# CIAM-Group/ComputerVision_Codes

Hardware: AMD Instinct MI355X
Metric: frames/sec spatial-extract + per-video TCN latency, Cholec80, 1/2/4/8 GPU (higher is better)
Workload: dtype bf16

## Files before the change

### computervision_codes_amd/csrc/bottleneck_fused.hip

```cpp
#include "mt4_common.h"

typedef __bf16 bf16x8_t __attribute__((ext_vector_type(8)));

namespace {

constexpr int TH = 8, TW = 14, NHALO = 160, NPX = 128;
constexpr int ROW_B = 128;
constexpr int XS_BYTES = NHALO * ROW_B;
constexpr int T2_BYTES = NPX * ROW_B;
constexpr int T1_BYTES = XS_BYTES + 2 * ROW_B;
constexpr int YS_BYTES = NPX * 256;

struct BneckK {
    const char* x;
    char* y;
    const char *w1, *w2, *w3, *wds;
    const float *b1, *b2, *b3, *bds;
    int B, H, W, tiles_h, tiles_w;
    int nt;
    char* y2;
    const char* wn;
    const float* bn;
    int H2, W2;
};

__device__ __forceinline__ f32x4 bias4(const float* b, int n) {
    const float4 t = *(const float4*)(b + n);
    return (f32x4){t.x, t.y, t.z, t.w};
}

__device__ __forceinline__ uint2 relu_pack4(f32x4 v) {
    uint2 o = make_uint2(pack_bf16x2(v[0], v[1]), pack_bf16x2(v[2], v[3]));
    asm("v_pk_max_i16 %0, %0, 0" : "+v"(o.x));
    asm("v_pk_max_i16 %0, %0, 0" : "+v"(o.y));
    return o;
}

__device__ __forceinline__ f32x4 mfma_bf16(uint4 wfrag, uint4 xfrag, f32x4 acc) {
    return __builtin_amdgcn_mfma_f32_16x16x32_bf16(__builtin_bit_cast(bf16x8_t, wfrag), __builtin_bit_cast(bf16x8_t, xfrag), acc, 0, 0, 0);
}

template <int CIN, bool DS, bool NEXT = false>
__global__ __launch_bounds__(256, 2) void bottleneck64_fused_kernel(const BneckK a) {
    static_assert(!NEXT || !DS, "the following conv rides behind an identity block");
    constexpr int KC = CIN / 64;
    constexpr int NXS = KC > 1 ? 2 : 1;
    static_assert(DS ? CIN == 64 : CIN == 256, "layer1.0 (64 channels in, downsample branch) or layer1.1+ (256 in, identity)");
    extern __shared__ __attribute__((aligned(16))) char smem[];
    char* const xs = smem;
    char* const t2 = smem + NXS * XS_BYTES;
    char* const t1 = t2 + T2_BYTES;
    char* const ys = DS ? t1 : xs;

    const int tid = threadIdx.x;
    const int lane = tid & 63, wave = tid >> 6;
    const int r16 = lane & 15, q = lane >> 4;

    int bid = blockIdx.x;
    {
        const int nb = gridDim.x;
        const int q8 = nb >> 3, r8 = nb & 7;
        const int xcd = bid & 7, local = bid >> 3;
        bid = (xcd < r8 ? xcd * (q8 + 1) : r8 * (q8 + 1) + (xcd - r8) * q8) + local;
    }
    const int tpi = a.tiles_h * a.tiles_w;
    const int img = bid / tpi;
    const int trem = bid - img * tpi;
    const int th = trem / a.tiles_w;
    const int h0 = th * TH, w0 = (trem - th * a.tiles_w) * TW;
    const char* const ximg = a.x + (long long)img * a.H * a.W * (CIN * 2);
    char* const yimg = NEXT ? a.y + (long long)img * a.H2 * a.W2 * 512 : a.y + (long long)img * a.H * a.W * 512;

    const int ld_row = tid >> 3, ld_chunk = tid & 7;
    int xoff[5];
#pragma unroll
    for (int i = 0; i < 5; ++i) {
        const int hp = ld_row + 32 * i;
        const int h = h0 - 1 + (hp >> 4), w = w0 - 1 + (hp & 15);
        xoff[i] = ((unsigned)h < (unsigned)a.H && (unsigned)w < (unsigned)a.W) ? (h * a.W + w) * (CIN * 2) + ld_chunk * 16 : -1;
    }
    auto load_chunk = [&](int kc, uint4 (&stg)[5]) {
#pragma unroll
        for (int i = 0; i < 5; ++i) {
            stg[i] = make_uint4(0, 0, 0, 0);
            if (xoff[i] >= 0) stg[i] = *(const uint4*)(ximg + xoff[i] + kc * 128);
        }
    };
    auto store_chunk = [&](int buf, const uint4 (&stg)[5]) {
#pragma unroll
        for (int i = 0; i < 5; ++i) {
            const int hp = ld_row + 32 * i;
            *(uint4*)(xs + buf * XS_BYTES + hp * ROW_B + ((ld_chunk ^ (hp & 7)) << 4)) = stg[i];
        }
    };
    uint4 stg0[5], stg1[5];
    load_chunk(0, stg0);
    if constexpr (KC > 1) load_chunk(1, stg1);

    const int ch1 = wave * 16;
    uint4 wf1[KC * 2];
    {
        const char* wr = a.w1 + (wave * (KC * 2) * 64 + lane) * 16;
#pragma unroll
        for (int s = 0; s < KC * 2; ++s) wf1[s] = *(const uint4*)(wr + s * 1024);
    }
    f32x4 acc1[10];
    {
        const f32x4 b4 = bias4(a.b1, ch1 + q * 4);
#pragma unroll
        for (int i = 0; i < 10; ++i) acc1[i] = b4;
    }
    const int sw0 = (q ^ (r16 & 7)) << 4, sw1 = ((4 + q) ^ (r16 & 7)) << 4;
    uint2 res[DS ? 1 : 4][DS ? 1 : 8];
    const int res_off = (r16 + 1) * ROW_B + (((2 * wave + (q >> 1)) ^ ((r16 + 1) & 7)) << 4) + (q & 1) * 8;
#pragma unroll
    for (int kc = 0; kc < KC; ++kc) {
        if (kc & 1) store_chunk(1, stg1); else store_chunk(0, stg0);
        if (kc + 2 < KC) { if (kc & 1) load_chunk(kc + 2, stg1); else load_chunk(kc + 2, stg0); }
        __syncthreads();
        const char* sb = xs + (kc & 1) * XS_BYTES + r16 * ROW_B;
        uint4 fx[2][10];
#pragma unroll
        for (int kk = 0; kk < 2; ++kk)
#pragma unroll
            for (int i = 0; i < 10; ++i) fx[kk][i] = *(const uint4*)(sb + i * 16 * ROW_B + (kk ? sw1 : sw0));
        if constexpr (!DS) {
#pragma unroll
            for (int j = 0; j < 8; ++j) res[kc][j] = *(const uint2*)(xs + (kc & 1) * XS_BYTES + (j + 1) * (16 * ROW_B) + res_off);
        }
        asm volatile("" ::: "memory");
#pragma unroll
        for (int kk = 0; kk < 2; ++kk)
#pragma unroll
            for (int i = 0; i < 10; ++i) acc1[i] = mfma_bf16(wf1[kc * 2 + kk], fx[kk][i], acc1[i]);
    }
    uint4 wf2[18];
    {
        const char* wr = a.w2 + (wave * 18 * 64 + lane) * 16;
#pragma unroll
        for (int s = 0; s < 18; ++s) wf2[s] = *(const uint4*)(wr + s * 1024);
    }
    const int cb1 = (ch1 + q * 4) * 2;
    {
        const int wr_off = r16 * ROW_B + (((cb1 >> 4) ^ (r16 & 7)) << 4) + (cb1 & 8);
        const int w = w0 - 1 + r16;
#pragma unroll
        for (int i = 0; i < 10; ++i) {
            const int h = h0 - 1 + i;
            const bool in = (unsigned)h < (unsigned)a.H && (unsigned)w < (unsigned)a.W;
            uint2 o = make_uint2(0, 0);
            if (in) o = relu_pack4(acc1[i]);
            *(uint2*)(t1 + i * (16 * ROW_B) + wr_off) = o;
        }
    }
    __syncthreads();

    f32x4 acc2[8];
    {
        const f32x4 b4 = bias4(a.b2, ch1 + q * 4);
#pragma unroll
        for (int j = 0; j < 8; ++j) acc2[j] = b4;
    }
    int toff[3][2];
#pragma unroll
    for (int kw = 0; kw < 3; ++kw)
#pragma unroll
        for (int kk = 0; kk < 2; ++kk) toff[kw][kk] = (r16 + kw) * ROW_B + (((kk * 4 + q) ^ ((r16 + kw) & 7)) << 4);
#pragma unroll
    for (int hr = 0; hr < 10; ++hr) {
        uint4 fr[3][2];
#pragma unroll
        for (int kw = 0; kw < 3; ++kw)
#pragma unroll
            for (int kk = 0; kk < 2; ++kk) fr[kw][kk] = *(const uint4*)(t1 + hr * (16 * ROW_B) + toff[kw][kk]);
        asm volatile("" ::: "memory");
#pragma unroll
        for (int kh = 0; kh < 3; ++kh) {
            const int ty = hr - kh;
            if (ty >= 0 && ty < 8) {
#pragma unroll
                for (int kw = 0; kw < 3; ++kw)
#pragma unroll
                    for (int kk = 0; kk < 2; ++kk) acc2[ty] = mfma_bf16(wf2[(kh * 3 + kw) * 2 + kk], fr[kw][kk], acc2[ty]);
            }
        }
    }
    uint4 wf3[4][2];
    uint4 wfd[DS ? 4 : 1][2];
#pragma unroll
    for (int i = 0; i < 4; ++i) {
        const char* wr = a.w3 + ((4 * i + wave) * 2 * 64 + lane) * 16;
        wf3[i][0] = *(const uint4*)wr;
        wf3[i][1] = *(const uint4*)(wr + 1024);
        if constexpr (DS) {
            const char* wd = a.wds + ((4 * i + wave) * 2 * 64 + lane) * 16;
            wfd[i][0] = *(const uint4*)wd;
            wfd[i][1] = *(const uint4*)(wd + 1024);
        }
    }
    {
        const int wr_off = r16 * ROW_B + (((cb1 >> 4) ^ (r16 & 7)) << 4) + (cb1 & 8);
#pragma unroll
        for (int j = 0; j < 8; ++j) {
            const uint2 o = relu_pack4(acc2[j]);
            *(uint2*)(t2 + j * (16 * ROW_B) + wr_off) = o;
        }
    }
    __syncthreads();

    uint4 fx3[8][2];
#pragma unroll
    for (int j = 0; j < 8; ++j) {
        fx3[j][0] = *(const uint4*)(t2 + j * (16 * ROW_B) + r16 * ROW_B + sw0);
        fx3[j][1] = *(const uint4*)(t2 + j * (16 * ROW_B) + r16 * ROW_B + sw1);
    }
    const int st_tx = tid >> 4, st_chunk = tid & 15;
    uint4 wfn[NEXT ? 2 : 1][NEXT ? 8 : 1];
#pragma unroll
    for (int pass = 0; pass < 2; ++pass) {
        char* const ysp = NEXT ? xs + pass * YS_BYTES : ys;
        if (pass && !NEXT) __syncthreads();
#pragma unroll
        for (int ii = 0; ii < 2; ++ii) {
            const int i = pass * 2 + ii;
            const int ct = 4 * i + wave;
            f32x4 acc3[8];
            {
                const f32x4 b4 = bias4(a.b3, ct * 16 + q * 4);
#pragma unroll
                for (int j = 0; j < 8; ++j) acc3[j] = b4;
            }
#pragma unroll
            for (int kk = 0; kk < 2; ++kk)
#pragma unroll
                for (int j = 0; j < 8; ++j) acc3[j] = mfma_bf16(wf3[i][kk], fx3[j][kk], acc3[j]);
            if constexpr (DS) {
                const f32x4 bd4 = bias4(a.bds, ct * 16 + q * 4);
#pragma unroll
                for (int j = 0; j < 8; ++j) {
                    f32x4 accd = bd4;
#pragma unroll
                    for (int kk = 0; kk < 2; ++kk) accd = mfma_bf16(wfd[i][kk], *(const uint4*)(xs + (j + 1) * (16 * ROW_B) + toff[1][kk]), accd);
#pragma unroll
                    for (int e = 0; e < 4; ++e) acc3[j][e] += bf16_to_f32(f32_to_bf16(accd[e]));
                }
            } else {
#pragma unroll
                for (int j = 0; j < 8; ++j) {
                    acc3[j][0] += __uint_as_float(res[i][j].x << 16);
                    acc3[j][1] += __uint_as_float(res[i][j].x & 0xffff0000u);
                    acc3[j][2] += __uint_as_float(res[i][j].y << 16);
                    acc3[j][3] += __uint_as_float(res[i][j].y & 0xffff0000u);
                }
            }
            const int cbyte = ((ct - 8 * pass) * 16 + q * 4) * 2;
            const int wr_off = r16 * 256 + (((cbyte >> 4) ^ r16) << 4) + (cbyte & 8);
#pragma unroll
            for (int j = 0; j < 8; ++j) {
                const uint2 o = relu_pack4(acc3[j]);
                *(uint2*)(ysp + j * (16 * 256) + wr_off) = o;
            }
        }
        if constexpr (NEXT) {
            if (pass == 1) {
#pragma unroll
                for (int c = 0; c < 2; ++c)
#pragma unroll
                    for (int ks = 0; ks < 8; ++ks) wfn[c][ks] = *(const uint4*)(a.wn + (((2 * wave + c) * 8 + ks) * 64 + lane) * 16);
            }
        }
        __syncthreads();
        {
            const int w = w0 + st_tx;
            const int rd_off = st_tx * 256 + ((st_chunk ^ st_tx) << 4);
            if constexpr (NEXT) {
                if (st_tx < TW && w < a.W && !(st_tx & 1)) {
                    const uint4 v0 = *(const uint4*)(ysp + rd_off), v1 = *(const uint4*)(ysp + 2 * (16 * 256) + rd_off);
                    const uint4 v2 = *(const uint4*)(ysp + 4 * (16 * 256) + rd_off), v3 = *(const uint4*)(ysp + 6 * (16 * 256) + rd_off);
                    char* const yp = yimg + (unsigned)(((h0 >> 1) * a.W2 + (w >> 1)) * 512 + pass * 256 + st_chunk * 16);
                    const int rows = a.H - h0;
                    *(uint4*)yp = v0;
                    if (rows > 2) *(uint4*)(yp + a.W2 * 512) = v1;
                    if (rows > 4) *(uint4*)(yp + 2 * a.W2 * 512) = v2;
                    if (rows > 6) *(uint4*)(yp + 3 * a.W2 * 512) = v3;
                }
            } else if (st_tx < TW && w < a.W) {
                uint4 v[8];
#pragma unroll
                for (int ty = 0; ty < 8; ++ty) v[ty] = *(const uint4*)(ysp + ty * (16 * 256) + rd_off);
                asm volatile("" ::: "memory");
#pragma unroll
                for (int ty = 0; ty < 8; ++ty) {
                    if (h0 + ty < a.H) {
                        typedef unsigned u32x4 __attribute__((ext_vector_type(4)));
                        char* yp = yimg + (unsigned)((h0 + ty) * a.W * 512) + (unsigned)(w * 512 + pass * 256 + st_chunk * 16);
                        if (a.nt) __builtin_nontemporal_store((u32x4){v[ty].x, v[ty].y, v[ty].z, v[ty].w}, (u32x4*)yp);
                        else *(uint4*)yp = v[ty];
                    }
                }
            }
        }
    }
    if constexpr (NEXT) {
        f32x4 acc4[2][8];
#pragma unroll
        for (int c = 0; c < 2; ++c) {
            const f32x4 b4 = bias4(a.bn, (2 * wave + c) * 16 + q * 4);
#pragma unroll
            for (int j = 0; j < 8; ++j) acc4[c][j] = b4;
        }
#pragma unroll
        for (int ks = 0; ks < 8; ++ks) {
            uint4 fy[8];
            const char* yb = xs + (ks >> 2) * YS_BYTES + r16 * 256 + ((((ks & 3) * 4 + q) ^ r16) << 4);
#pragma unroll
            for (int j = 0; j < 8; ++j) fy[j] = *(const uint4*)(yb + j * (16 * 256));
            asm volatile("" ::: "memory");
#pragma unroll
            for (int c = 0; c < 2; ++c)
#pragma unroll
                for (int j = 0; j < 8; ++j) acc4[c][j] = mfma_bf16(wfn[c][ks], fy[j], acc4[c][j]);
        }
        __syncthreads();
#pragma unroll
        for (int c = 0; c < 2; ++c) {
            const int cbyte = ((2 * wave + c) * 16 + q * 4) * 2;
            const int wr_off = r16 * 256 + (((cbyte >> 4) ^ r16) << 4) + (cbyte & 8);
#pragma unroll
            for (int j = 0; j < 8; ++j) *(uint2*)(xs + j * (16 * 256) + wr_off) = relu_pack4(acc4[c][j]);
        }
        __syncthreads();
        const int w = w0 + st_tx;
        if (st_tx < TW && w < a.W) {
            const int rd_off = st_tx * 256 + ((st_chunk ^ st_tx) << 4);
            char* const y2img = a.y2 + (long long)img * a.H * a.W * 256;
            uint4 v[8];
#pragma unroll
            for (int ty = 0; ty < 8; ++ty) v[ty] = *(const uint4*)(xs + ty * (16 * 256) + rd_off);
            asm volatile("" ::: "memory");
#pragma unroll
            for (int ty = 0; ty < 8; ++ty) {
                if (h0 + ty < a.H) {
                    typedef unsigned u32x4 __attribute__((ext_vector_type(4)));
                    char* yp = y2img + (unsigned)(((h0 + ty) * a.W + w) * 256 + st_chunk * 16);
                    if (a.nt) __builtin_nontemporal_store((u32x4){v[ty].x, v[ty].y, v[ty].z, v[ty].w}, (u32x4*)yp);
                    else *(uint4*)yp = v[ty];
                }
            }
        }
    }
}

template <int CIN, bool DS, bool NEXT = false>
int launch(const BneckK& a, hipStream_t stream) {
    constexpr int NXS = CIN > 64 ? 2 : 1;
    constexpr int LDS = NXS * XS_BYTES + T2_BYTES + (DS ? YS_BYTES : T1_BYTES);
    static_assert(LDS <= 80 * 1024, "two workgroups per CU");
    static_assert(!NEXT || LDS >= 2 * YS_BYTES, "both output passes stay in LDS");
    auto fn = bottleneck64_fused_kernel<CIN, DS, NEXT>;
    MT4_RAISE_LDS(fn);
    const long long nblk = (long long)a.B * a.tiles_h * a.tiles_w;
    hipLaunchKernelGGL(fn, dim3((unsigned)nblk), dim3(256), LDS, stream, a);
    return mt4_check_launch();
}

}

__global__ void bneck_pack_kernel(const u16* __restrict__ w, uint4* __restrict__ out, int ctiles, int ksteps, int row_elems) {
    const int i = blockIdx.x * blockDim.x + threadIdx.x;
    if (i >= ctiles * ksteps * 64) return;
    const int lane = i & 63, fs = i >> 6;
    const int step = fs % ksteps, tile = fs / ksteps;
    out[i] = *(const uint4*)(w + (long long)(tile * 16 + (lane & 15)) * row_elems + step * 32 + (lane >> 4) * 8);
}

static inline long long bneck_frag_bytes(int Cin, bool ds) { return ((long long)4 * (Cin / 32) + 4 * 18 + 16 * 2 + (ds ? 16 * (Cin / 32) : 0)) * 1024; }

extern "C" int64_t mt4_bottleneck_packed_bytes(int32_t Cin, int32_t has_downsample) {
    if (!((has_downsample && Cin == 64) || (!has_downsample && Cin == 256))) return MT4_EUNSUPPORTED;
    return bneck_frag_bytes(Cin, has_downsample != 0);
}

extern "C" int mt4_bottleneck_pack_bf16(const void* w1, const void* w2, const void* w3, const void* wds, int32_t Cin, void* out, void* stream) {
    mt4_clear_error();
    if (!w1 || !w2 || !w3 || !out) return MT4_EINVAL;
    if (!((wds && Cin == 64) || (!wds && Cin == 256))) return MT4_EUNSUPPORTED;
    if (((uintptr_t)w1 | (uintptr_t)w2 | (uintptr_t)w3 | (uintptr_t)wds | (uintptr_t)out) & 15) return MT4_EALIGN;
    hipStream_t s = (hipStream_t)stream;
    const int k1 = Cin / 32;
    char* o = (char*)out;
    const int r1 = (int)mt4_conv_packed_k(Cin, 1, 1, MT4_BF16), r2 = (int)mt4_conv_packed_k(64, 3, 3, MT4_BF16), r3 = (int)mt4_conv_packed_k(64, 1, 1, MT4_BF16);
    auto go = [&](const void* w, int ctiles, int ksteps, int row_elems) {
        const int n = ctiles * ksteps * 64;
        hipLaunchKernelGGL(bneck_pack_kernel, dim3((n + 255) / 256), dim3(256), 0, s, (const u16*)w, (uint4*)o, ctiles, ksteps, row_elems);
        o += (long long)n * 16;
    };
    go(w1, 4, k1, r1);
    go(w2, 4, 18, r2);
    go(w3, 16, 2, r3);
    if (wds) go(wds, 16, k1, r1);
    return mt4_check_launch();
}

extern "C" int mt4_bottleneck_fused_bf16(const void* x, void* y, const void* w_frag, const float* b1, const float* b2, const float* b3, const float* bds,
                                         int32_t B, int32_t H, int32_t W, int32_t Cin, int32_t mid, void* stream) {
    mt4_clear_error();
    if (!x || !y || !w_frag || !b1 || !b2 || !b3 || B <= 0 || H <= 0 || W <= 0) return MT4_EINVAL;
    const bool ds = bds != nullptr;
    if (mid != 64 || !((ds && Cin == 64) || (!ds && Cin == 256))) return MT4_EUNSUPPORTED;
    if (((uintptr_t)x | (uintptr_t)y | (uintptr_t)w_frag | (uintptr_t)b1 | (uintptr_t)b2 | (uintptr_t)b3 | (uintptr_t)bds) & 15) return MT4_EALIGN;
    if ((long long)H * W * 512 > 0x7fffffffLL) return MT4_EUNSUPPORTED;
    BneckK a;
    a.x = (const char*)x; a.y = (char*)y;
    const int k1 = Cin / 32;
    a.w1 = (const char*)w_frag;
    a.w2 = a.w1 + (long long)4 * k1 * 1024;
    a.w3 = a.w2 + (long long)4 * 18 * 1024;
    a.wds = ds ? a.w3 + (long long)16 * 2 * 1024 : nullptr;
    a.b1 = b1; a.b2 = b2; a.b3 = b3; a.bds = bds;
    a.B = B; a.H = H; a.W = W;
    a.tiles_h = cdiv(H, TH); a.tiles_w = cdiv(W, TW);
    a.nt = 1;
    if ((long long)B * a.tiles_h * a.tiles_w > 0x7fffffffLL) return MT4_EUNSUPPORTED;
    return ds ? launch<64, true>(a, (hipStream_t)stream) : launch<256, false>(a, (hipStream_t)stream);
}

extern "C" int64_t mt4_bottleneck_next_packed_bytes(void) { return (int64_t)8 * 8 * 1024; }

extern "C" int mt4_bottleneck_pack_next_bf16(const void* w1_next, void* out, void* stream) {
    mt4_clear_error();
    if (!w1_next || !out) return MT4_EINVAL;
    if (((uintptr_t)w1_next | (uintptr_t)out) & 15) return MT4_EALIGN;
    const int n = 8 * 8 * 64;
    hipLaunchKernelGGL(bneck_pack_kernel, dim3((n + 255) / 256), dim3(256), 0, (hipStream_t)stream, (const u16*)w1_next, (uint4*)out, 8, 8,
                       (int)mt4_conv_packed_k(256, 1, 1, MT4_BF16));
    return mt4_check_launch();
}

extern "C" int mt4_bottleneck_fused_next_bf16(const void* x, void* y_even, void* t_next, const void* w_frag, const float* b1, const float* b2,
                                              const float* b3, const void* w_next, const float* b_next, int32_t B, int32_t H, int32_t W, void* stream) {
    mt4_clear_error();
    if (!x || !y_even || !t_next || !w_frag || !b1 || !b2 || !b3 || !w_next || !b_next || B <= 0 || H <= 0 || W <= 0) return MT4_EINVAL;
    if (((uintptr_t)x | (uintptr_t)y_even | (uintptr_t)t_next | (uintptr_t)w_frag | (uintptr_t)b1 | (uintptr_t)b2 | (uintptr_t)b3 | (uintptr_t)w_next |
         (uintptr_t)b_next) & 15)
        return MT4_EALIGN;
    if ((long long)H * W * 512 > 0x7fffffffLL) return MT4_EUNSUPPORTED;
    BneckK a{};
    a.x = (const char*)x; a.y = (char*)y_even; a.y2 = (char*)t_next;
    a.w1 = (const char*)w_frag;
    a.w2 = a.w1 + (long long)4 * 8 * 1024;
    a.w3 = a.w2 + (long long)4 * 18 * 1024;
    a.wds = nullptr;
    a.b1 = b1; a.b2 = b2; a.b3 = b3; a.bds = nullptr;
    a.wn = (const char*)w_next; a.bn = b_next;
    a.B = B; a.H = H; a.W = W; a.H2 = (H + 1) / 2; a.W2 = (W + 1) / 2;
    a.tiles_h = cdiv(H, TH); a.tiles_w = cdiv(W, TW);
    a.nt = 1;
    if ((long long)B * a.tiles_h * a.tiles_w > 0x7fffffffLL) return MT4_EUNSUPPORTED;
    return launch<256, false, true>(a, (hipStream_t)stream);
}

extern "C" int mt4_pack_fragments_bf16(const void* w_packed, int32_t rows, int32_t row_elems, void* out, void* stream) {
    mt4_clear_error();
    if (!w_packed || !out || rows <= 0 || row_elems <= 0) return MT4_EINVAL;
    if ((rows % 16) || (row_elems % 32)) return MT4_EUNSUPPORTED;
    if (((uintptr_t)w_packed | (uintptr_t)out) & 15) return MT4_EALIGN;
    const long long n = (long long)(rows / 16) * (row_elems / 32) * 64;
    if (n > 0x7fffffffLL) return MT4_EUNSUPPORTED;
    hipLaunchKernelGGL(bneck_pack_kernel, dim3((unsigned)((n + 255) / 256)), dim3(256), 0, (hipStream_t)stream, (const u16*)w_packed, (uint4*)out, rows / 16,
                       row_elems / 32, row_elems);
    return mt4_check_launch();
}
```

Before: 97370.

## Process vertical strips of tiles per workgroup, carrying conv1 halo rows between bands

Each workgroup now walks a vertical strip of up to several 8x14 tiles instead of one tile. The two halo rows of the 1x1 conv output and the residual row are carried in LDS and registers to the next band, so recomputing the halo conv1 rows and reloading the overlapping input rows is avoided. It reduces the redundant 10-vs-8 row work and the halo reads, at the cost of fewer workgroups (with a floor of 1024 blocks), more serialization per block and extra LDS for the DS variant.

```diff
diff --git a/computervision_codes_amd/csrc/bottleneck_fused.hip b/computervision_codes_amd/csrc/bottleneck_fused.hip
--- a/computervision_codes_amd/csrc/bottleneck_fused.hip
+++ b/computervision_codes_amd/csrc/bottleneck_fused.hip
@@ -17,6 +17,7 @@
     const char *w1, *w2, *w3, *wds;
     const float *b1, *b2, *b3, *bds;
     int B, H, W, tiles_h, tiles_w;
+    int strips_h, bands;
     int nt;
     char* y2;
     const char* wn;
@@ -39,6 +40,8 @@
 __device__ __forceinline__ f32x4 mfma_bf16(uint4 wfrag, uint4 xfrag, f32x4 acc) {
     return __builtin_amdgcn_mfma_f32_16x16x32_bf16(__builtin_bit_cast(bf16x8_t, wfrag), __builtin_bit_cast(bf16x8_t, xfrag), acc, 0, 0, 0);
 }
+
+template <int N> struct Tag { static constexpr int v = N; };
 
 template <int CIN, bool DS, bool NEXT = false>
 __global__ __launch_bounds__(256, 2) void bottleneck64_fused_kernel(const BneckK a) {
@@ -53,8 +56,6 @@
     char* const ys = DS ? t1 : xs;
 
     const int tid = threadIdx.x;
-    const int lane = tid & 63, wave = tid >> 6;
-    const int r16 = lane & 15, q = lane >> 4;
 
     int bid = blockIdx.x;
     {
@@ -63,305 +64,352 @@
         const int xcd = bid & 7, local = bid >> 3;
         bid = (xcd < r8 ? xcd * (q8 + 1) : r8 * (q8 + 1) + (xcd - r8) * q8) + local;
     }
-    const int tpi = a.tiles_h * a.tiles_w;
-    const int img = bid / tpi;
-    const int trem = bid - img * tpi;
-    const int th = trem / a.tiles_w;
-    const int h0 = th * TH, w0 = (trem - th * a.tiles_w) * TW;
+    const int spi = a.strips_h * a.tiles_w;
+    const int img = bid / spi;
+    const int srem = bid - img * spi;
+    const int sh = srem / a.tiles_w;
+    const int w0 = (srem - sh * a.tiles_w) * TW;
+    const int band0 = sh * a.bands;
+    const int nband = min(a.bands, a.tiles_h - band0);
     const char* const ximg = a.x + (long long)img * a.H * a.W * (CIN * 2);
     char* const yimg = NEXT ? a.y + (long long)img * a.H2 * a.W2 * 512 : a.y + (long long)img * a.H * a.W * 512;
 
-    const int ld_row = tid >> 3, ld_chunk = tid & 7;
-    int xoff[5];
-#pragma unroll
-    for (int i = 0; i < 5; ++i) {
-        const int hp = ld_row + 32 * i;
-        const int h = h0 - 1 + (hp >> 4), w = w0 - 1 + (hp & 15);
-        xoff[i] = ((unsigned)h < (unsigned)a.H && (unsigned)w < (unsigned)a.W) ? (h * a.W + w) * (CIN * 2) + ld_chunk * 16 : -1;
-    }
-    auto load_chunk = [&](int kc, uint4 (&stg)[5]) {
-#pragma unroll
-        for (int i = 0; i < 5; ++i) {
-            stg[i] = make_uint4(0, 0, 0, 0);
-            if (xoff[i] >= 0) stg[i] = *(const uint4*)(ximg + xoff[i] + kc * 128);
-        }
-    };
-    auto store_chunk = [&](int buf, const uint4 (&stg)[5]) {
-#pragma unroll
-        for (int i = 0; i < 5; ++i) {
+#define BNECK_LANE_VARS(t)                                                                                                              \
+    const int lane = (t) & 63, wave = (t) >> 6;                                                                                       \
+    const int r16 = lane & 15, q = lane >> 4;                                                                                          \
+    const int ch1 = wave * 16;                                                                 \
+    const int cb1 = (ch1 + q * 4) * 2;                                    \
+    const int sw0 = (q ^ (r16 & 7)) << 4, sw1 = ((4 + q) ^ (r16 & 7)) << 4;        \
+    (void)cb1; (void)sw0; (void)sw1
+    uint2 carry[DS ? 1 : 4];
+    uint2 res[DS ? 1 : 4][DS ? 1 : 8];
+
+    auto phase1 = [&](auto pro, int h0) {
+        int t = tid;
+        asm volatile("" : "+v"(t));
+        BNECK_LANE_VARS(t);
+        const int ld_row = t >> 3, ld_chunk = t & 7;
+        const int res_off = (r16 + 1) * ROW_B + (((2 * wave + (q >> 1)) ^ ((r16 + 1) & 7)) << 4) + (q & 1) * 8;
+        constexpr bool PRO = decltype(pro)::v != 0;
+        constexpr int NR = PRO ? 2 : TH;
+        constexpr int XR0 = (DS && !PRO) ? 1 : 0;
+        constexpr int NP = ((NR + XR0) * 16 + 31) / 32;
+        const int hx0 = PRO ? h0 - 1 : h0 + 1 - XR0;
+        int xoff[NP];
+#pragma unroll
+        for (int i = 0; i < NP; ++i) {
             const int hp = ld_row + 32 * i;
-            *(uint4*)(xs + buf * XS_BYTES + hp * ROW_B + ((ld_chunk ^ (hp & 7)) << 4)) = stg[i];
-        }
-    };
-    uint4 stg0[5], stg1[5];
-    load_chunk(0, stg0);
-    if constexpr (KC > 1) load_chunk(1, stg1);
-
-    const int ch1 = wave * 16;
-    uint4 wf1[KC * 2];
-    {
-        const char* wr = a.w1 + (wave * (KC * 2) * 64 + lane) * 16;
-#pragma unroll
-        for (int s = 0; s < KC * 2; ++s) wf1[s] = *(const uint4*)(wr + s * 1024);
-    }
-    f32x4 acc1[10];
-    {
-        const f32x4 b4 = bias4(a.b1, ch1 + q * 4);
-#pragma unroll
-        for (int i = 0; i < 10; ++i) acc1[i] = b4;
-    }
-    const int sw0 = (q ^ (r16 & 7)) << 4, sw1 = ((4 + q) ^ (r16 & 7)) << 4;
-    uint2 res[DS ? 1 : 4][DS ? 1 : 8];
-    const int res_off = (r16 + 1) * ROW_B + (((2 * wave + (q >> 1)) ^ ((r16 + 1) & 7)) << 4) + (q & 1) * 8;
-#pragma unroll
-    for (int kc = 0; kc < KC; ++kc) {
-        if (kc & 1) store_chunk(1, stg1); else store_chunk(0, stg0);
-        if (kc + 2 < KC) { if (kc & 1) load_chunk(kc + 2, stg1); else load_chunk(kc + 2, stg0); }
-        __syncthreads();
-        const char* sb = xs + (kc & 1) * XS_BYTES + r16 * ROW_B;
-        uint4 fx[2][10];
-#pragma unroll
-        for (int kk = 0; kk < 2; ++kk)
-#pragma unroll
-            for (int i = 0; i < 10; ++i) fx[kk][i] = *(const uint4*)(sb + i * 16 * ROW_B + (kk ? sw1 : sw0));
-        if constexpr (!DS) {
-#pragma unroll
-            for (int j = 0; j < 8; ++j) res[kc][j] = *(const uint2*)(xs + (kc & 1) * XS_BYTES + (j + 1) * (16 * ROW_B) + res_off);
-        }
-        asm volatile("" ::: "memory");
-#pragma unroll
-        for (int kk = 0; kk < 2; ++kk)
-#pragma unroll
-            for (int i = 0; i < 10; ++i) acc1[i] = mfma_bf16(wf1[kc * 2 + kk], fx[kk][i], acc1[i]);
-    }
-    uint4 wf2[18];
-    {
-        const char* wr = a.w2 + (wave * 18 * 64 + lane) * 16;
-#pragma unroll
-        for (int s = 0; s < 18; ++s) wf2[s] = *(const uint4*)(wr + s * 1024);
-    }
-    const int cb1 = (ch1 + q * 4) * 2;
-    {
+            const int h = hx0 + (hp >> 4), w = w0 - 1 + (hp & 15);
+            xoff[i] = (hp < (NR + XR0) * 16 && (unsigned)h < (unsigned)a.H && (unsigned)w < (unsigned)a.W) ? (h * a.W + w) * (CIN * 2) + ld_chunk * 16 : -1;
+        }
+        auto load_chunk = [&](int kc, uint4 (&stg)[NP]) {
+#pragma unroll
+            for (int i = 0; i < NP; ++i) {
+                stg[i] = make_uint4(0, 0, 0, 0);
+                if (xoff[i] >= 0) stg[i] = *(const uint4*)(ximg + xoff[i] + kc * 128);
+            }
+        };
+        auto store_chunk = [&](int buf, const uint4 (&stg)[NP]) {
+#pragma unroll
+            for (int i = 0; i < NP; ++i) {
+                const int hp = ld_row + 32 * i;
+                *(uint4*)(xs + buf * XS_BYTES + hp * ROW_B + ((ld_chunk ^ (hp & 7)) << 4)) = stg[i];
+            }
+        };
+        uint4 stg0[NP], stg1[NP];
+        load_chunk(0, stg0);
+        if constexpr (KC > 1) load_chunk(1, stg1);
+        uint4 wf1[KC * 2];
+        {
+            const char* wr = a.w1 + (wave * (KC * 2) * 64 + lane) * 16;
+#pragma unroll
+            for (int s = 0; s < KC * 2; ++s) wf1[s] = *(const uint4*)(wr + s * 1024);
+        }
+        f32x4 acc1[NR];
+        {
+            const f32x4 b4 = bias4(a.b1, ch1 + q * 4);
+#pragma unroll
+            for (int i = 0; i < NR; ++i) acc1[i] = b4;
+        }
+#pragma unroll
+        for (int kc = 0; kc < KC; ++kc) {
+            if (kc & 1) store_chunk(1, stg1); else store_chunk(0, stg0);
+            if (kc + 2 < KC) { if (kc & 1) load_chunk(kc + 2, stg1); else load_chunk(kc + 2, stg0); }
+            __syncthreads();
+            const char* xb = xs + (kc & 1) * XS_BYTES;
+            const char* sb = xb + (XR0 * 16 + r16) * ROW_B;
+            uint4 fx[2][NR];
+#pragma unroll
+            for (int kk = 0; kk < 2; ++kk)
+#pragma unroll
+                for (int i = 0; i < NR; ++i) fx[kk][i] = *(const uint4*)(sb + i * 16 * ROW_B + (kk ? sw1 : sw0));
+            if constexpr (!DS) {
+                if constexpr (PRO) {
+                    carry[kc] = *(const uint2*)(xb + 1 * (16 * ROW_B) + res_off);
+                } else {
+                    res[kc][0] = carry[kc];
+#pragma unroll
+                    for (int j = 1; j < TH; ++j) res[kc][j] = *(const uint2*)(xb + (j - 1) * (16 * ROW_B) + res_off);
+                    carry[kc] = *(const uint2*)(xb + (TH - 1) * (16 * ROW_B) + res_off);
+                }
+            }
+            asm volatile("" ::: "memory");
+#pragma unroll
+            for (int kk = 0; kk < 2; ++kk)
+#pragma unroll
+                for (int i = 0; i < NR; ++i) acc1[i] = mfma_bf16(wf1[kc * 2 + kk], fx[kk][i], acc1[i]);
+        }
         const int wr_off = r16 * ROW_B + (((cb1 >> 4) ^ (r16 & 7)) << 4) + (cb1 & 8);
         const int w = w0 - 1 + r16;
 #pragma unroll
-        for (int i = 0; i < 10; ++i) {
-            const int h = h0 - 1 + i;
+        for (int i = 0; i < NR; ++i) {
+            const int h = hx0 + XR0 + i;
             const bool in = (unsigned)h < (unsigned)a.H && (unsigned)w < (unsigned)a.W;
             uint2 o = make_uint2(0, 0);
             if (in) o = relu_pack4(acc1[i]);
-            *(uint2*)(t1 + i * (16 * ROW_B) + wr_off) = o;
-        }
-    }
+            *(uint2*)(t1 + ((PRO ? 0 : 2) + i) * (16 * ROW_B) + wr_off) = o;
+        }
+    };
+
+    char* const t1c = DS ? ys + YS_BYTES : t1 + 8 * (16 * ROW_B);
+    phase1(Tag<1>(), band0 * TH);
     __syncthreads();
-
-    f32x4 acc2[8];
-    {
-        const f32x4 b4 = bias4(a.b2, ch1 + q * 4);
-#pragma unroll
-        for (int j = 0; j < 8; ++j) acc2[j] = b4;
-    }
-    int toff[3][2];
-#pragma unroll
-    for (int kw = 0; kw < 3; ++kw)
-#pragma unroll
-        for (int kk = 0; kk < 2; ++kk) toff[kw][kk] = (r16 + kw) * ROW_B + (((kk * 4 + q) ^ ((r16 + kw) & 7)) << 4);
-#pragma unroll
-    for (int hr = 0; hr < 10; ++hr) {
-        uint4 fr[3][2];
+#pragma clang loop unroll(disable)
+    for (int bi = 0; bi < nband; ++bi) {
+        const int h0 = (band0 + bi) * TH;
+        int t = tid;
+        asm volatile("" : "+v"(t));
+        if (bi) *(uint4*)(t1 + t * 16) = *(const uint4*)(t1c + t * 16);
+        phase1(Tag<0>(), h0);
+        BNECK_LANE_VARS(t);
+        uint4 wf2[18];
+        {
+            const char* wr = a.w2 + (wave * 18 * 64 + lane) * 16;
+#pragma unroll
+            for (int s = 0; s < 18; ++s) wf2[s] = *(const uint4*)(wr + s * 1024);
+        }
+        __syncthreads();
+
+        f32x4 acc2[8];
+        {
+            const f32x4 b4 = bias4(a.b2, ch1 + q * 4);
+#pragma unroll
+            for (int j = 0; j < 8; ++j) acc2[j] = b4;
+        }
+        int toff[3][2];
 #pragma unroll
         for (int kw = 0; kw < 3; ++kw)
 #pragma unroll
-            for (int kk = 0; kk < 2; ++kk) fr[kw][kk] = *(const uint4*)(t1 + hr * (16 * ROW_B) + toff[kw][kk]);
-        asm volatile("" ::: "memory");
-#pragma unroll
-        for (int kh = 0; kh < 3; ++kh) {
-            const int ty = hr - kh;
-            if (ty >= 0 && ty < 8) {
-#pragma unroll
-                for (int kw = 0; kw < 3; ++kw)
-#pragma unroll
-                    for (int kk = 0; kk < 2; ++kk) acc2[ty] = mfma_bf16(wf2[(kh * 3 + kw) * 2 + kk], fr[kw][kk], acc2[ty]);
-            }
-        }
-    }
-    uint4 wf3[4][2];
-    uint4 wfd[DS ? 4 : 1][2];
-#pragma unroll
-    for (int i = 0; i < 4; ++i) {
-        const char* wr = a.w3 + ((4 * i + wave) * 2 * 64 + lane) * 16;
-        wf3[i][0] = *(const uint4*)wr;
-        wf3[i][1] = *(const uint4*)(wr + 1024);
-        if constexpr (DS) {
-            const char* wd = a.wds + ((4 * i + wave) * 2 * 64 + lane) * 16;
-            wfd[i][0] = *(const uint4*)wd;
-            wfd[i][1] = *(const uint4*)(wd + 1024);
-        }
-    }
-    {
-        const int wr_off = r16 * ROW_B + (((cb1 >> 4) ^ (r16 & 7)) << 4) + (cb1 & 8);
+            for (int kk = 0; kk < 2; ++kk) toff[kw][kk] = (r16 + kw) * ROW_B + (((kk * 4 + q) ^ ((r16 + kw) & 7)) << 4);
+#pragma unroll
+        for (int hr = 0; hr < 10; ++hr) {
+            uint4 fr[3][2];
+#pragma unroll
+            for (int kw = 0; kw < 3; ++kw)
+#pragma unroll
+                for (int kk = 0; kk < 2; ++kk) fr[kw][kk] = *(const uint4*)(t1 + hr * (16 * ROW_B) + toff[kw][kk]);
+            asm volatile("" ::: "memory");
+#pragma unroll
+            for (int kh = 0; kh < 3; ++kh) {
+                const int ty = hr - kh;
+                if (ty >= 0 && ty < 8) {
+#pragma unroll
+                    for (int kw = 0; kw < 3; ++kw)
+#pragma unroll
+                        for (int kk = 0; kk < 2; ++kk) acc2[ty] = mfma_bf16(wf2[(kh * 3 + kw) * 2 + kk], fr[kw][kk], acc2[ty]);
+                }
+            }
+        }
+        if constexpr (DS) *(uint4*)(t1c + t * 16) = *(const uint4*)(t1 + 8 * (16 * ROW_B) + t * 16);
+        uint4 wf3[4][2];
+        uint4 wfd[DS ? 4 : 1][2];
+#pragma unroll
+        for (int i = 0; i < 4; ++i) {
+            const char* wr = a.w3 + ((4 * i + wave) * 2 * 64 + lane) * 16;
+            wf3[i][0] = *(const uint4*)wr;
+            wf3[i][1] = *(const uint4*)(wr + 1024);
+            if constexpr (DS) {
+                const char* wd = a.wds + ((4 * i + wave) * 2 * 64 + lane) * 16;
+                wfd[i][0] = *(const uint4*)wd;
+                wfd[i][1] = *(const uint4*)(wd + 1024);
+            }
+        }
+        {
+            const int wr_off = r16 * ROW_B + (((cb1 >> 4) ^ (r16 & 7)) << 4) + (cb1 & 8);
+#pragma unroll
+            for (int j = 0; j < 8; ++j) {
+                const uint2 o = relu_pack4(acc2[j]);
+                *(uint2*)(t2 + j * (16 * ROW_B) + wr_off) = o;
+            }
+        }
+        __syncthreads();
+
+        uint4 fx3[8][2];
 #pragma unroll
         for (int j = 0; j < 8; ++j) {
-            const uint2 o = relu_pack4(acc2[j]);
-            *(uint2*)(t2 + j * (16 * ROW_B) + wr_off) = o;
-        }
-    }
-    __syncthreads();
-
-    uint4 fx3[8][2];
-#pragma unroll
-    for (int j = 0; j < 8; ++j) {
-        fx3[j][0] = *(const uint4*)(t2 + j * (16 * ROW_B) + r16 * ROW_B + sw0);
-        fx3[j][1] = *(const uint4*)(t2 + j * (16 * ROW_B) + r16 * ROW_B + sw1);
-    }
-    const int st_tx = tid >> 4, st_chunk = tid & 15;
-    uint4 wfn[NEXT ? 2 : 1][NEXT ? 8 : 1];
-#pragma unroll
-    for (int pass = 0; pass < 2; ++pass) {
-        char* const ysp = NEXT ? xs + pass * YS_BYTES : ys;
-        if (pass && !NEXT) __syncthreads();
-#pragma unroll
-        for (int ii = 0; ii < 2; ++ii) {
-            const int i = pass * 2 + ii;
-            const int ct = 4 * i + wave;
-            f32x4 acc3[8];
+            fx3[j][0] = *(const uint4*)(t2 + j * (16 * ROW_B) + r16 * ROW_B + sw0);
+            fx3[j][1] = *(const uint4*)(t2 + j * (16 * ROW_B) + r16 * ROW_B + sw1);
+        }
+        const int st_tx = t >> 4, st_chunk = t & 15;
+        uint4 wfn[NEXT ? 2 : 1][NEXT ? 8 : 1];
+#pragma unroll
+        for (int pass = 0; pass < 2; ++pass) {
+            char* const ysp = NEXT ? xs + pass * YS_BYTES : ys;
+            if (pass && !NEXT) __syncthreads();
+#pragma unroll
+            for (int ii = 0; ii < 2; ++ii) {
+                const int i = pass * 2 + ii;
+                const int ct = 4 * i + wave;
+                f32x4 acc3[8];
+                {
+                    const f32x4 b4 = bias4(a.b3, ct * 16 + q * 4);
+#pragma unroll
+                    for (int j = 0; j < 8; ++j) acc3[j] = b4;
+                }
+#pragma unroll
+                for (int kk = 0; kk < 2; ++kk)
+#pragma unroll
+                    for (int j = 0; j < 8; ++j) acc3[j] = mfma_bf16(wf3[i][kk], fx3[j][kk], acc3[j]);
+                if constexpr (DS) {
+                    const f32x4 bd4 = bias4(a.bds, ct * 16 + q * 4);
+#pragma unroll
+                    for (int j = 0; j < 8; ++j) {
+                        f32x4 accd = bd4;
+#pragma unroll
+                        for (int kk = 0; kk < 2; ++kk) accd = mfma_bf16(wfd[i][kk], *(const uint4*)(xs + j * (16 * ROW_B) + toff[1][kk]), accd);
+#pragma unroll
+                        for (int e = 0; e < 4; ++e) acc3[j][e] += bf16_to_f32(f32_to_bf16(accd[e]));
+                    }
+                } else {
+#pragma unroll
+                    for (int j = 0; j < 8; ++j) {
+                        acc3[j][0] += __uint_as_float(res[i][j].x << 16);
+                        acc3[j][1] += __uint_as_float(res[i][j].x & 0xffff0000u);
+                        acc3[j][2] += __uint_as_float(res[i][j].y << 16);
+                        acc3[j][3] += __uint_as_float(res[i][j].y & 0xffff0000u);
+                    }
+                }
+                const int cbyte = ((ct - 8 * pass) * 16 + q * 4) * 2;
+                const int wr_off = r16 * 256 + (((cbyte >> 4) ^ r16) << 4) + (cbyte & 8);
+#pragma unroll
+                for (int j = 0; j < 8; ++j) {
+                    const uint2 o = relu_pack4(acc3[j]);
+                    *(uint2*)(ysp + j * (16 * 256) + wr_off) = o;
+                }
+            }
+            if constexpr (NEXT) {
+                if (pass == 1) {
+#pragma unroll
+                    for (int c = 0; c < 2; ++c)
+#pragma unroll
+                        for (int ks = 0; ks < 8; ++ks) wfn[c][ks] = *(const uint4*)(a.wn + (((2 * wave + c) * 8 + ks) * 64 + lane) * 16);
+                }
+            }
+            __syncthreads();
             {
-                const f32x4 b4 = bias4(a.b3, ct * 16 + q * 4);
-#pragma unroll
-                for (int j = 0; j < 8; ++j) acc3[j] = b4;
-            }
-#pragma unroll
-            for (int kk = 0; kk < 2; ++kk)
-#pragma unroll
-                for (int j = 0; j < 8; ++j) acc3[j] = mfma_bf16(wf3[i][kk], fx3[j][kk], acc3[j]);
-            if constexpr (DS) {
-                const f32x4 bd4 = bias4(a.bds, ct * 16 + q * 4);
-#pragma unroll
-                for (int j = 0; j < 8; ++j) {
-                    f32x4 accd = bd4;
-#pragma unroll
-                    for (int kk = 0; kk < 2; ++kk) accd = mfma_bf16(wfd[i][kk], *(const uint4*)(xs + (j + 1) * (16 * ROW_B) + toff[1][kk]), accd);
-#pragma unroll
-                    for (int e = 0; e < 4; ++e) acc3[j][e] += bf16_to_f32(f32_to_bf16(accd[e]));
-                }
-            } else {
-#pragma unroll
-                for (int j = 0; j < 8; ++j) {
-                    acc3[j][0] += __uint_as_float(res[i][j].x << 16);
-                    acc3[j][1] += __uint_as_float(res[i][j].x & 0xffff0000u);
-                    acc3[j][2] += __uint_as_float(res[i][j].y << 16);
-                    acc3[j][3] += __uint_as_float(res[i][j].y & 0xffff0000u);
-                }
-            }
-            const int cbyte = ((ct - 8 * pass) * 16 + q * 4) * 2;
-            const int wr_off = r16 * 256 + (((cbyte >> 4) ^ r16) << 4) + (cbyte & 8);
-#pragma unroll
-            for (int j = 0; j < 8; ++j) {
-                const uint2 o = relu_pack4(acc3[j]);
-                *(uint2*)(ysp + j * (16 * 256) + wr_off) = o;
+                const int w = w0 + st_tx;
+                const int rd_off = st_tx * 256 + ((st_chunk ^ st_tx) << 4);
+                if constexpr (NEXT) {
+                    if (st_tx < TW && w < a.W && !(st_tx & 1)) {
+                        const uint4 v0 = *(const uint4*)(ysp + rd_off), v1 = *(const uint4*)(ysp + 2 * (16 * 256) + rd_off);
+                        const uint4 v2 = *(const uint4*)(ysp + 4 * (16 * 256) + rd_off), v3 = *(const uint4*)(ysp + 6 * (16 * 256) + rd_off);
+                        char* const yp = yimg + (unsigned)(((h0 >> 1) * a.W2 + (w >> 1)) * 512 + pass * 256 + st_chunk * 16);
+                        const int rows = a.H - h0;
+                        *(uint4*)yp = v0;
+                        if (rows > 2) *(uint4*)(yp + a.W2 * 512) = v1;
+                        if (rows > 4) *(uint4*)(yp + 2 * a.W2 * 512) = v2;
+                        if (rows > 6) *(uint4*)(yp + 3 * a.W2 * 512) = v3;
+                    }
+                } else if (st_tx < TW && w < a.W) {
+                    uint4 v[8];
+#pragma unroll
+                    for (int ty = 0; ty < 8; ++ty) v[ty] = *(const uint4*)(ysp + ty * (16 * 256) + rd_off);
+                    asm volatile("" ::: "memory");
+#pragma unroll
+                    for (int ty = 0; ty < 8; ++ty) {
+                        if (h0 + ty < a.H) {
+                            typedef unsigned u32x4 __attribute__((ext_vector_type(4)));
+                            char* yp = yimg + (unsigned)((h0 + ty) * a.W * 512) + (unsigned)(w * 512 + pass * 256 + st_chunk * 16);
+                            if (a.nt) __builtin_nontemporal_store((u32x4){v[ty].x, v[ty].y, v[ty].z, v[ty].w}, (u32x4*)yp);
+                            else *(uint4*)yp = v[ty];
+                        }
+                    }
+                }
             }
         }
         if constexpr (NEXT) {
-            if (pass == 1) {
+            f32x4 acc4[2][8];
+#pragma unroll
+            for (int c = 0; c < 2; ++c) {
+                const f32x4 b4 = bias4(a.bn, (2 * wave + c) * 16 + q * 4);
+#pragma unroll
+                for (int j = 0; j < 8; ++j) acc4[c][j] = b4;
+            }
+#pragma unroll
+            for (int ks = 0; ks < 8; ++ks) {
+                uint4 fy[8];
+                const char* yb = xs + (ks >> 2) * YS_BYTES + r16 * 256 + ((((ks & 3) * 4 + q) ^ r16) << 4);
+#pragma unroll
+                for (int j = 0; j < 8; ++j) fy[j] = *(const uint4*)(yb + j * (16 * 256));
+                asm volatile("" ::: "memory");
 #pragma unroll
                 for (int c = 0; c < 2; ++c)
 #pragma unroll
-                    for (int ks = 0; ks < 8; ++ks) wfn[c][ks] = *(const uint4*)(a.wn + (((2 * wave + c) * 8 + ks) * 64 + lane) * 16);
-            }
-        }
-        __syncthreads();
-        {
+                    for (int j = 0; j < 8; ++j) acc4[c][j] = mfma_bf16(wfn[c][ks], fy[j], acc4[c][j]);
+            }
+            __syncthreads();
+#pragma unroll
+            for (int c = 0; c < 2; ++c) {
+                const int cbyte = ((2 * wave + c) * 16 + q * 4) * 2;
+                const int wr_off = r16 * 256 + (((cbyte >> 4) ^ r16) << 4) + (cbyte & 8);
+#pragma unroll
+                for (int j = 0; j < 8; ++j) *(uint2*)(xs + j * (16 * 256) + wr_off) = relu_pack4(acc4[c][j]);
+            }
+            __syncthreads();
             const int w = w0 + st_tx;
-            const int rd_off = st_tx * 256 + ((st_chunk ^ st_tx) << 4);
-            if constexpr (NEXT) {
-                if (st_tx < TW && w < a.W && !(st_tx & 1)) {
-                    const uint4 v0 = *(const uint4*)(ysp + rd_off), v1 = *(const uint4*)(ysp + 2 * (16 * 256) + rd_off);
-                    const uint4 v2 = *(const uint4*)(ysp + 4 * (16 * 256) + rd_off), v3 = *(const uint4*)(ysp + 6 * (16 * 256) + rd_off);
-                    char* const yp = yimg + (unsigned)(((h0 >> 1) * a.W2 + (w >> 1)) * 512 + pass * 256 + st_chunk * 16);
-                    const int rows = a.H - h0;
-                    *(uint4*)yp = v0;
-                    if (rows > 2) *(uint4*)(yp + a.W2 * 512) = v1;
-                    if (rows > 4) *(uint4*)(yp + 2 * a.W2 * 512) = v2;
-                    if (rows > 6) *(uint4*)(yp + 3 * a.W2 * 512) = v3;
-                }
-            } else if (st_tx < TW && w < a.W) {
+            if (st_tx < TW && w < a.W) {
+                const int rd_off = st_tx * 256 + ((st_chunk ^ st_tx) << 4);
+                char* const y2img = a.y2 + (long long)img * a.H * a.W * 256;
                 uint4 v[8];
 #pragma unroll
-                for (int ty = 0; ty < 8; ++ty) v[ty] = *(const uint4*)(ysp + ty * (16 * 256) + rd_off);
+                for (int ty = 0; ty < 8; ++ty) v[ty] = *(const uint4*)(xs + ty * (16 * 256) + rd_off);
                 asm volatile("" ::: "memory");
 #pragma unroll
                 for (int ty = 0; ty < 8; ++ty) {
                     if (h0 + ty < a.H) {
                         typedef unsigned u32x4 __attribute__((ext_vector_type(4)));
-                        char* yp = yimg + (unsigned)((h0 + ty) * a.W * 512) + (unsigned)(w * 512 + pass * 256 + st_chunk * 16);
+                        char* yp = y2img + (unsigned)(((h0 + ty) * a.W + w) * 256 + st_chunk * 16);
                         if (a.nt) __builtin_nontemporal_store((u32x4){v[ty].x, v[ty].y, v[ty].z, v[ty].w}, (u32x4*)yp);
                         else *(uint4*)yp = v[ty];
                     }
                 }
             }
         }
+        __syncthreads();
     }
-    if constexpr (NEXT) {
-        f32x4 acc4[2][8];
-#pragma unroll
-        for (int c = 0; c < 2; ++c) {
-            const f32x4 b4 = bias4(a.bn, (2 * wave + c) * 16 + q * 4);
-#pragma unroll
-            for (int j = 0; j < 8; ++j) acc4[c][j] = b4;
-        }
-#pragma unroll
-        for (int ks = 0; ks < 8; ++ks) {
-            uint4 fy[8];
-            const char* yb = xs + (ks >> 2) * YS_BYTES + r16 * 256 + ((((ks & 3) * 4 + q) ^ r16) << 4);
-#pragma unroll
-            for (int j = 0; j < 8; ++j) fy[j] = *(const uint4*)(yb + j * (16 * 256));
-            asm volatile("" ::: "memory");
-#pragma unroll
-            for (int c = 0; c < 2; ++c)
-#pragma unroll
-                for (int j = 0; j < 8; ++j) acc4[c][j] = mfma_bf16(wfn[c][ks], fy[j], acc4[c][j]);
-        }
-        __syncthreads();
-#pragma unroll
-        for (int c = 0; c < 2; ++c) {
-            const int cbyte = ((2 * wave + c) * 16 + q * 4) * 2;
-            const int wr_off = r16 * 256 + (((cbyte >> 4) ^ r16) << 4) + (cbyte & 8);
-#pragma unroll
-            for (int j = 0; j < 8; ++j) *(uint2*)(xs + j * (16 * 256) + wr_off) = relu_pack4(acc4[c][j]);
-        }
-        __syncthreads();
-        const int w = w0 + st_tx;
-        if (st_tx < TW && w < a.W) {
-            const int rd_off = st_tx * 256 + ((st_chunk ^ st_tx) << 4);
-            char* const y2img = a.y2 + (long long)img * a.H * a.W * 256;
-            uint4 v[8];
-#pragma unroll
-            for (int ty = 0; ty < 8; ++ty) v[ty] = *(const uint4*)(xs + ty * (16 * 256) + rd_off);
-            asm volatile("" ::: "memory");
-#pragma unroll
-            for (int ty = 0; ty < 8; ++ty) {
-                if (h0 + ty < a.H) {
-                    typedef unsigned u32x4 __attribute__((ext_vector_type(4)));
-                    char* yp = y2img + (unsigned)(((h0 + ty) * a.W + w) * 256 + st_chunk * 16);
-                    if (a.nt) __builtin_nontemporal_store((u32x4){v[ty].x, v[ty].y, v[ty].z, v[ty].w}, (u32x4*)yp);
-                    else *(uint4*)yp = v[ty];
-                }
-            }
-        }
-    }
+#undef BNECK_LANE_VARS
 }
 
 template <int CIN, bool DS, bool NEXT = false>
 int launch(const BneckK& a, hipStream_t stream) {
     constexpr int NXS = CIN > 64 ? 2 : 1;
-    constexpr int LDS = NXS * XS_BYTES + T2_BYTES + (DS ? YS_BYTES : T1_BYTES);
+    constexpr int LDS = NXS * XS_BYTES + T2_BYTES + (DS ? YS_BYTES + 2 * 16 * ROW_B : T1_BYTES);
     static_assert(LDS <= 80 * 1024, "two workgroups per CU");
     static_assert(!NEXT || LDS >= 2 * YS_BYTES, "both output passes stay in LDS");
+    static_assert(DS || NXS * XS_BYTES + T2_BYTES + 8 * (16 * ROW_B) >= (NEXT ? 2 : 1) * YS_BYTES, "the output staging leaves t1 rows 8, 9 alone");
     auto fn = bottleneck64_fused_kernel<CIN, DS, NEXT>;
     MT4_RAISE_LDS(fn);
-    const long long nblk = (long long)a.B * a.tiles_h * a.tiles_w;
+    const long long nblk = (long long)a.B * a.strips_h * a.tiles_w;
     hipLaunchKernelGGL(fn, dim3((unsigned)nblk), dim3(256), LDS, stream, a);
     return mt4_check_launch();
+}
+
+constexpr int MAX_BANDS = 7;
+void set_strips(BneckK& a) {
+    a.tiles_h = cdiv(a.H, TH); a.tiles_w = cdiv(a.W, TW);
+    a.bands = cdiv(a.tiles_h, cdiv(a.tiles_h, MAX_BANDS));
+    while (a.bands > 1 && (long long)a.B * a.tiles_w * cdiv(a.tiles_h, a.bands) < 1024) a.bands = cdiv(a.bands, 2);
+    a.strips_h = cdiv(a.tiles_h, a.bands);
 }
 
 }
@@ -419,9 +467,9 @@
     a.wds = ds ? a.w3 + (long long)16 * 2 * 1024 : nullptr;
     a.b1 = b1; a.b2 = b2; a.b3 = b3; a.bds = bds;
     a.B = B; a.H = H; a.W = W;
-    a.tiles_h = cdiv(H, TH); a.tiles_w = cdiv(W, TW);
+    set_strips(a);
     a.nt = 1;
-    if ((long long)B * a.tiles_h * a.tiles_w > 0x7fffffffLL) return MT4_EUNSUPPORTED;
+    if ((long long)B * a.strips_h * a.tiles_w > 0x7fffffffLL) return MT4_EUNSUPPORTED;
     return ds ? launch<64, true>(a, (hipStream_t)stream) : launch<256, false>(a, (hipStream_t)stream);
 }
 
@@ -454,9 +502,9 @@
     a.b1 = b1; a.b2 = b2; a.b3 = b3; a.bds = nullptr;
     a.wn = (const char*)w_next; a.bn = b_next;
     a.B = B; a.H = H; a.W = W; a.H2 = (H + 1) / 2; a.W2 = (W + 1) / 2;
-    a.tiles_h = cdiv(H, TH); a.tiles_w = cdiv(W, TW);
+    set_strips(a);
     a.nt = 1;
-    if ((long long)B * a.tiles_h * a.tiles_w > 0x7fffffffLL) return MT4_EUNSUPPORTED;
+    if ((long long)B * a.strips_h * a.tiles_w > 0x7fffffffLL) return MT4_EUNSUPPORTED;
     return launch<256, false, true>(a, (hipStream_t)stream);
 }
 
```

Result: no change. 97600 (median of 6 runs) (+0.2%).
